# mjmyt/drone_path_planning_python

Hardware: AMD Instinct MI355X
Metric: minimum-snap trajectories/sec (N drones × M segments, order 7) at 1/2/4/8 MI355X (higher is better)
Workload: dtype f64

## Files before the change

### drone_path_planning_python_amd/csrc/msnap_aux.hip

```cpp
#include <math.h>

#include <cstdlib>

#include "msnap_internal.h"

namespace msnap {

__global__ void __launch_bounds__(256)
pack_kernel(const double *__restrict__ coef, const double *__restrict__ dur, float *__restrict__ out,
            size_t n_rows , int nc) {
  const int ncol = 1 + 4 * nc;
  const size_t total = n_rows * (size_t)ncol;
  for (size_t idx = (size_t)blockIdx.x * blockDim.x + threadIdx.x; idx < total;
       idx += (size_t)gridDim.x * blockDim.x) {
    const size_t row = idx / ncol;
    const int col = (int)(idx - row * ncol);
    const double v = (col == 0) ? dur[row] : coef[row * (size_t)(4 * nc) + (col - 1)];
    out[idx] = (float)v;
  }
}

int launch_pack(msnap_ctx *ctx, int n_drones, int n_seg, const double *coef, const double *dur, float *out) {
  const size_t rows = (size_t)n_drones * n_seg;
  const int nc = ctx->order + 1;
// ... 1262 lines not shown
        if (keep && pos < cg.cap) {
          const int a = a0 + ai, b = a + t * kSelThreads + threadIdx.x;
          cg.glist[pos] = (a << 16) | b;
          if (b != a) cg.blist[(size_t)b * cg.nG + a] = pos + 1;
        }
      }
    return;
  }
  constexpr int GPB = kRowBlock / kColBlock;
  constexpr int NW = kSelThreads / kWave;
  __shared__ int wsum[kSelTrips][NW];
  __shared__ int sStart;
  __shared__ double sRow[GPB][8];
  __shared__ double sAll[8];
  const int I = blockIdx.x, lane = threadIdx.x & (kWave - 1), w = threadIdx.x / kWave;
  const int nsh = (N - I * kRowBlock + kColBlock - 1) / kColBlock;
  const int ng = nsh < GPB ? nsh : GPB;
  if (threadIdx.x < 7 * GPB) {
    const int q = threadIdx.x / 7, k = threadIdx.x % 7;
    if (q < ng) sRow[q][k] = k < 6 ? (kStage ? sBox[(I * GPB + q) * 6 + k] : cu.colbox[(size_t)(I * GPB + q) * 6 + k]) : sCmax[I * GPB + q];
  }
  __syncthreads();
  if (threadIdx.x < 7) {
    const int k = threadIdx.x;
    double v = sRow[0][k];
    for (int q = 1; q < ng; ++q) v = k < 3 ? fmin(v, sRow[q][k]) : fmax(v, sRow[q][k]);
    sAll[k] = v;
  }
  __syncthreads();
  unsigned long long mk[kSelTrips];
  bool keep[kSelTrips];
  double cbx[kSelTrips][6], cmx[kSelTrips];
#pragma unroll
  for (int t = 0; t < kSelTrips; ++t) {
    if (t * kSelThreads >= nsh) continue;
    const int k = t * kSelThreads + threadIdx.x, J = I * GPB + (k < nsh ? k : nsh - 1);
    load_box(J, cbx[t]);
    cmx[t] = sCmax[J];
  }
#pragma unroll
  for (int t = 0; t < kSelTrips; ++t) {
    const int k = t * kSelThreads + threadIdx.x;
    keep[t] = false;
    if (k < nsh) {
      keep[t] = true;
      if (k >= GPB) {
        const double cm = cmx[t];
        bool any = false;
        const double lb0 = box_box_lb2(sAll, cbx[t]);
        if (!((lb0 > sAll[6]) & (lb0 > cm))) {
          for (int q = 0; q < ng; ++q) {
            const double lb2 = box_box_lb2(sRow[q], cbx[t]);
            any |= !((lb2 > sRow[q][6]) & (lb2 > cm));
          }
        }
        keep[t] = any;
      }
    }
    mk[t] = __ballot(keep[t]);
    if (lane == 0) wsum[t][w] = __popcll(mk[t]);
  }
  __syncthreads();
  int all = 0, off[kSelTrips];
#pragma unroll
  for (int t = 0; t < kSelTrips; ++t) {
#pragma unroll
    for (int q = 0; q < NW; ++q) {
      if (q == w) off[t] = all;
      all += wsum[t][q];
    }
  }
  if (threadIdx.x == 0) {
    const int start = atomicAdd(&meta[kMetaTotal], all);
    sStart = start;
    meta[kMetaStart + I] = start;
    cnt[I] = all;
  }
  __syncthreads();
#pragma unroll
  for (int t = 0; t < kSelTrips; ++t)
    if (keep[t]) list[sStart + off[t] + __popcll(mk[t] & ((1ull << lane) - 1ull))] = (I << 16) | (t * kSelThreads + threadIdx.x);
}

__device__ __forceinline__ void
collide_span_list_body(const double *__restrict__ prow_t, const double *__restrict__ pcol, CollideGeom g,
                       double *__restrict__ part_d2, int32_t *__restrict__ part_j, double *__restrict__ cpart_d2,
                       int32_t *__restrict__ cpart_i, const int32_t *__restrict__ oid, const int32_t *__restrict__ list,
                       int sp_force, int slots, int32_t *__restrict__ meta) {
  constexpr int CB = kColBlock;
  __shared__ double sFold[CB * kWave];
  __shared__ int sFoldI[CB * kWave];
  const int lane = threadIdx.x;
  const int tot = meta[kMetaTotal];
  const CullSplit sp = cull_split(tot, slots, cull_nch(g.S), sp_force);
  if (blockIdx.x == 0 && lane == 0) {
    meta[kMetaParts] = sp.lo;
    meta[kMetaParts + 1] = sp.hi;
    meta[kMetaParts + 2] = sp.x;
  }
  const int items = sp.items(tot);
  const int xi = sp.x * sp.hi;
  auto share_of = [&](int it) { return it < xi ? it / sp.hi : sp.x + (it - xi) / sp.lo; };
  int it = blockIdx.x;
  int entry = it < items ? list[share_of(it)] : 0;
  while (it < items) {
    const int f = share_of(it);
    g.sparts = it < xi ? sp.hi : sp.lo;
    const int h = it - sp.item_of(f);
    const int I = entry >> 16, k = entry & 0xffff;
    const int nxt = it + gridDim.x;
    entry = nxt < items ? list[share_of(nxt)] : 0;
    const int crow = I * sp.hi + h;
    const int cj = I * kRowBlock + k * CB;
    const int ncols = g.Cn - cj < CB ? g.Cn - cj : CB;
    const bool two_sided = k >= kRowBlock / CB;
    RowSet rs;
#pragma unroll
    for (int rr = 0; rr < kRowsPerLane; ++rr) {
      const int raw = I * kRowBlock + rr * kWave + lane;
      rs.live[rr] = raw < g.R;
      rs.grow[rr] = rs.live[rr] ? raw : g.R - 1;
      rs.best[rr] = INFINITY;
      rs.bestj[rr] = -1;
    }
    const double *prowT = prow_t + (size_t)I * kRowBlock;
    if (ncols <= 2)
      collide_block<2, true>(g, prowT, pcol, cj, ncols, two_sided, rs, I, h, crow, lane, sFold, sFoldI, cpart_d2, cpart_i, oid);
    else if (ncols <= CB / 2)
      collide_block<CB / 2, true>(g, prowT, pcol, cj, ncols, two_sided, rs, I, h, crow, lane, sFold, sFoldI, cpart_d2, cpart_i, oid);
    else
      collide_block<CB, true>(g, prowT, pcol, cj, ncols, two_sided, rs, I, h, crow, lane, sFold, sFoldI, cpart_d2, cpart_i, oid);
#pragma unroll
    for (int rr = 0; rr < kRowsPerLane; ++rr) {
      part_d2[(size_t)it * kRowBlock + rr * kWave + lane] = rs.best[rr];
      part_j[(size_t)it * kRowBlock + rr * kWave + lane] = (rs.best[rr] == INFINITY) ? -1 : rs.bestj[rr];
    }
    it = nxt;
  }
}

constexpr int kGroupHalf = kColBlock / 2;
constexpr int kGroupLanes = kWave / 2;

constexpr int kFinishWaves = 4;
template <int kChunks>
__global__ void __launch_bounds__(kWave * kFinishWaves)
collide_finish_groups_kernel(int N, const int32_t *__restrict__ oid, const int32_t *__restrict__ meta, CullGroups cg,
                             double radius, double *__restrict__ min_dist, int32_t *__restrict__ partner,
                             int32_t *__restrict__ hit) {
  __shared__ int sItAll[kFinishWaves][kChunks * kWave];
  const int lane = threadIdx.x & (kWave - 1), w = __builtin_amdgcn_readfirstlane(threadIdx.x / kWave);
  int *sIt = sItAll[w];
  const int gq = blockIdx.x * kFinishWaves + w;
  if (gq >= cg.nG || meta[kMetaGroups] > cg.cap) return;
  int pl[kChunks];
#pragma unroll
  for (int c = 0; c < kChunks; ++c)
    pl[c] = (c * kWave < gq && c * kWave + lane < gq) ? cg.blist[(size_t)gq * cg.nG + c * kWave + lane] : 0;
  const int nA = cg.acnt[gq], sA = cg.astart[gq];
  const int k = lane & (kColBlock - 1), e = lane >> 3;
  const int r = gq * kColBlock + k;
  const int out = r < N ? oid[r] : 0;
  int nB = 0;
#pragma unroll
  for (int c = 0; c < kChunks; ++c) {
    const unsigned long long m = __ballot(pl[c] > 0);
    if (pl[c] > 0) sIt[nB + __popcll(m & ((1ull << lane) - 1ull))] = pl[c] - 1;
    nB += __popcll(m);
  }
  __builtin_amdgcn_fence(__ATOMIC_RELEASE, "wavefront", "local");
  __builtin_amdgcn_wave_barrier();
  __builtin_amdgcn_fence(__ATOMIC_ACQUIRE, "wavefront", "local");
  double best = INFINITY;
  int bj = -1;
  constexpr int U = 8;
  for (int q0 = 0; q0 < nA + nB; q0 += U * (kWave / kColBlock)) {
    double d[U];
    int j[U];
#pragma unroll
    for (int u = 0; u < U; ++u) {
      const int q = q0 + u * (kWave / kColBlock) + e;
      d[u] = INFINITY;
      j[u] = -1;
      if (q < nA + nB) {
        const size_t slot = (q < nA ? (size_t)(sA + q) * 16 : (size_t)sIt[q - nA] * 16 + kColBlock) + k;
        d[u] = cg.cand_d2[slot];
        j[u] = cg.cand_j[slot];
      }
    }
#pragma unroll
    for (int u = 0; u < U; ++u)
      if (j[u] >= 0 && (bj < 0 || d[u] < best || (d[u] == best && j[u] < bj))) {
        best = d[u];
        bj = j[u];
      }
  }
#pragma unroll
  for (int m = kColBlock; m < kWave; m <<= 1) {
    const double o = shfl_xor_f64(best, m);
    const int oj = __shfl_xor(bj, m);
    if (oj >= 0 && (bj < 0 || o < best || (o == best && oj < bj))) {
      best = o;
      bj = oj;
    }
  }
  if (e == 0 && r < N) {
    const double dist = sqrt(bj >= 0 ? best : INFINITY);
    min_dist[out] = dist;
    partner[out] = bj;
    hit[out] = (dist < 2.0 * radius) ? 1 : 0;
  }
#pragma unroll
  for (int c = 0; c < kChunks; ++c)
    if (pl[c] > 0) cg.blist[(size_t)gq * cg.nG + c * kWave + lane] = 0;
}

constexpr int kGroupWaves = 4;
__global__ void __launch_bounds__(kWave, kGroupWaves)
collide_eval_groups_kernel(const double *__restrict__ pcol, int N, int S, const int32_t *__restrict__ oid,
                           const int32_t *__restrict__ meta, CullGroups cg, unsigned long long *__restrict__ hint) {
#pragma clang fp contract(off)
  const int lane = threadIdx.x;
  int tot = meta[kMetaGroups];
  if (blockIdx.x == 0 && lane == 0 && hint != nullptr)
    __hip_atomic_store(hint, cull_hint_pack(N, meta[kMetaTotal], tot), __ATOMIC_RELAXED, __HIP_MEMORY_SCOPE_SYSTEM);
  if (tot > cg.cap) tot = 0;
  const unsigned stride = (unsigned)S * 3u;
  const int per = (tot + 7) >> 3;
  auto item_of = [&](int v) { return (v >> 3) < per ? (v & 7) * per + (v >> 3) : tot; };
  int v = blockIdx.x, it = item_of(v);
  int entry = (it < tot && it < cg.cap) ? cg.glist[it] : 0;
  for (; (v >> 3) < per; v += gridDim.x, it = item_of(v)) {
    const int it_next = item_of(v + (int)gridDim.x);
    const int ent_raw = entry;
    entry = it_next < tot ? cg.glist[it_next] : 0;
    if (it >= tot) continue;
    const int ent = __builtin_amdgcn_readfirstlane(ent_raw);
    const int a = ent >> 16, b = ent & 0xffff;
    const bool diag = a == b;

    int lane_s = threadIdx.x;
    asm volatile("" : "+v"(lane_s));
    const int half = lane_s >> 5, ls = lane_s & (kGroupLanes - 1);
    double acc[kColBlock * kGroupHalf];
#pragma unroll
    for (int p = 0; p < kColBlock * kGroupHalf; ++p) acc[p] = INFINITY;
#pragma unroll 1
    for (int s0 = 0; s0 < S; s0 += kGroupLanes) {
      const int sq = s0 + ls < S ? s0 + ls : S - 1;
      const unsigned voff = (unsigned)sq * 24u;
      double cx[kGroupHalf], cy[kGroupHalf], cz[kGroupHalf];
#pragma unroll
      for (int c = 0; c < kGroupHalf; ++c) {
        const int d = b * kColBlock + half * kGroupHalf + c;
        const double *p = reinterpret_cast<const double *>(
            reinterpret_cast<const char *>(pcol + (size_t)(d < N ? d : N - 1) * stride) + (size_t)voff);
        cx[c] = p[0];
        cy[c] = p[1];
        cz[c] = p[2];
      }
      double rw[3][3];
      auto fetch = [&](int r, double(&dst)[3]) {
        const int d = a * kColBlock + r;
        const double *p = reinterpret_cast<const double *>(
            reinterpret_cast<const char *>(pcol + (size_t)(d < N ? d : N - 1) * stride) + (size_t)voff);
        dst[0] = p[0];
        dst[1] = p[1];
        dst[2] = p[2];
      };
      fetch(0, rw[0]);
      fetch(1, rw[1]);
#pragma unroll
      for (int r = 0; r < kColBlock; ++r) {
        if (r + 2 < kColBlock) fetch(r + 2, rw[(r + 2) % 3]);
        asm volatile("" ::: "memory");
        const double x = rw[r % 3][0], y = rw[r % 3][1], z = rw[r % 3][2];
#pragma unroll
        for (int c = 0; c < kGroupHalf; ++c) {
          const double dx = cx[c] - x, dy = cy[c] - y, dz = cz[c] - z;
          const double d2 = __builtin_fma(dz, dz, __builtin_fma(dy, dy, dx * dx));
          asm("v_min_f64 %0, %1, %0" : "+v"(acc[r * kGroupHalf + c]) : "v"(d2));
        }
      }
    }
#pragma unroll
    for (int n = 16, m = 16; n >= 1; n >>= 1, m >>= 1) {
      const bool up = (lane_s & m) != 0;
#pragma unroll
      for (int i = 0; i < n; ++i) {
        const double keep = up ? acc[i + n] : acc[i], send = up ? acc[i] : acc[i + n];
        acc[i] = __builtin_fmin(keep, __shfl_xor(send, m));
      }
    }
    double v = acc[0];
    int lane_c = threadIdx.x;
    asm volatile("" : "+v"(lane_c));
    const int pr = (lane_c & (kGroupLanes - 1)) >> 2, pc = lane_c & (kGroupHalf - 1), half_c = lane_c >> 5;
    const int ra = a * kColBlock + pr, cb = b * kColBlock + half_c * kGroupHalf + pc;
    const int oi = oid[ra < N ? ra : N - 1], oj = oid[cb < N ? cb : N - 1];
    if (ra >= N || cb >= N || (diag && ra == cb)) v = INFINITY;
    {
      double w = v;
      int wj = oj;
#pragma unroll
      for (int m = 1; m <= 32; m = (m == 2 ? 32 : m << 1)) {
        const double o = __shfl_xor(w, m);
        const int ojx = __shfl_xor(wj, m);
        const bool take = (o < w) | ((o == w) & (ojx < wj));
        w = take ? o : w;
        wj = take ? ojx : wj;
      }
      if ((lane & 35) == 0) {
        cg.cand_d2[(size_t)it * 16 + pr] = w;
        cg.cand_j[(size_t)it * 16 + pr] = w < INFINITY ? wj : -1;
      }
    }
    {
      double w = v;
      int wi = oi;
#pragma unroll
      for (int m = 4; m <= 16; m <<= 1) {
        const double o = __shfl_xor(w, m);
        const int oix = __shfl_xor(wi, m);
        const bool take = (o < w) | ((o == w) & (oix < wi));
        w = take ? o : w;
        wi = take ? oix : wi;
      }
      if ((lane_c & (kGroupLanes - 1)) < kGroupHalf) {
        const int k = kColBlock + half_c * kGroupHalf + pc;
        cg.cand_d2[(size_t)it * 16 + k] = w;
        cg.cand_j[(size_t)it * 16 + k] = (!diag && w < INFINITY) ? wi : -1;
      }
    }
  }
}

__global__ void __launch_bounds__(kWave, 4)
collide_eval_shares_kernel(const double *__restrict__ prow_t, const double *__restrict__ pcol, CollideGeom g,
                           double *__restrict__ part_d2, int32_t *__restrict__ part_j, double *__restrict__ cpart_d2,
                           int32_t *__restrict__ cpart_i, const int32_t *__restrict__ oid, const int32_t *__restrict__ list,
                           int sp_force, int slots, int32_t *__restrict__ meta, unsigned long long *__restrict__ hint,
                           int groups_cap) {
  if (groups_cap > 0 && meta[kMetaGroups] <= groups_cap) return;
  if (blockIdx.x == 0 && threadIdx.x == 0 && hint != nullptr)
    __hip_atomic_store(hint, cull_hint_pack(g.R, meta[kMetaTotal], meta[kMetaGroups]), __ATOMIC_RELAXED,
                       __HIP_MEMORY_SCOPE_SYSTEM);
  collide_span_list_body(prow_t, pcol, g, part_d2, part_j, cpart_d2, cpart_i, oid, list, sp_force, slots, meta);
}

__global__ void __launch_bounds__(kWave)
collide_short_kernel(const double *__restrict__ prow, const double *__restrict__ pcol, int R, int ro, int Cn, int S,
                     double radius, double *__restrict__ min_dist, int32_t *__restrict__ partner,
                     int32_t *__restrict__ hit, int raw) {
#pragma clang fp contract(off)
  const int r = blockIdx.x * kWave + threadIdx.x;
  if (r >= R) return;
  const int grow = ro + r;
  const double *pr = prow + (size_t)r * S * 3;
  double best = INFINITY;
  int bestj = -1;
  for (int j = 0; j < Cn; ++j) {
    const double *pc = pcol + (size_t)j * S * 3;
    double m = INFINITY;
    for (int sq = 0; sq < S; ++sq) {
      const double dx = pc[(size_t)sq * 3 + 0] - pr[(size_t)sq * 3 + 0];
      const double dy = pc[(size_t)sq * 3 + 1] - pr[(size_t)sq * 3 + 1];
      const double dz = pc[(size_t)sq * 3 + 2] - pr[(size_t)sq * 3 + 2];
      const double d2 = __builtin_fma(dz, dz, __builtin_fma(dy, dy, dx * dx));
      m = __builtin_fmin(d2, m);
    }
    if (j == grow) m = INFINITY;
    if (m < best) {
      best = m;
      bestj = j;
    }
  }
  if (raw) {
    min_dist[r] = best;
    partner[r] = (best == INFINITY) ? -1 : bestj;
    return;
  }
  const double dist = sqrt(best);
  min_dist[r] = dist;
  partner[r] = (best == INFINITY) ? -1 : bestj;
  hit[r] = (dist < 2.0 * radius) ? 1 : 0;
}

constexpr int kMergeRows = 16;
constexpr int kMergeParts = 16;
__global__ void __launch_bounds__(kMergeRows * kMergeParts)
collide_merge_kernel(const double *__restrict__ part_d2, const int32_t *__restrict__ part_j, CollideGeom g,
                     const double *__restrict__ cpart_d2, const int32_t *__restrict__ cpart_i, double radius,
                     double *__restrict__ min_dist, int32_t *__restrict__ partner, int32_t *__restrict__ hit,
                     const int32_t *__restrict__ oid, const int32_t *__restrict__ cnt, const int32_t *__restrict__ meta,
                     int groups_cap = 0) {
  if (groups_cap > 0 && meta[kMetaGroups] <= groups_cap) return;
  __shared__ double sD[kMergeParts][kMergeRows];
  __shared__ int sJ[kMergeParts][kMergeRows];
  const int lr = threadIdx.x & (kMergeRows - 1), q = threadIdx.x / kMergeRows;
  const int r_raw = blockIdx.x * kMergeRows + lr;
  const int r = r_raw < g.R ? r_raw : g.R - 1;
  const int out = oid ? oid[r] : r;
  double best = INFINITY;
  int bj = -1;
  constexpr int U = 8;
  auto sweep = [&](const double *pd, const int32_t *pj, size_t pitch, int n) {
    for (int s0 = q; s0 < n; s0 += U * kMergeParts) {
      double v[U];
      int j[U];
#pragma unroll
      for (int k = 0; k < U; ++k) {
        const int sidx = s0 + k * kMergeParts;
        const int sc = sidx < n ? sidx : n - 1;
        v[k] = pd[(size_t)sc * pitch];
        j[k] = sidx < n ? pj[(size_t)sc * pitch] : -1;
      }
#pragma unroll
      for (int k = 0; k < U; ++k) {
        if (j[k] >= 0 && (v[k] < best || (v[k] == best && j[k] < bj))) {
          best = v[k];
          bj = j[k];
        }
      }
    }
  };
  if (cnt) {
    const int I = __builtin_amdgcn_readfirstlane(r / kRowBlock);
    CullSplit sp;
    sp.lo = meta[kMetaParts];
    sp.hi = meta[kMetaParts + 1];
    sp.x = meta[kMetaParts + 2];
    const int f0 = meta[kMetaStart + I], first_item = sp.item_of(f0), n_items = sp.item_of(f0 + cnt[I]) - first_item;
    const size_t first = (size_t)first_item * kRowBlock + (r - I * kRowBlock);
    sweep(part_d2 + first, part_j + first, kRowBlock, n_items);
    if (I > 0) sweep(cpart_d2 + r, cpart_i + r, (size_t)g.R, I * sp.hi);
  } else if (g.total > 0) {
    const int I = r / kRowBlock;
    long long ua = collide_ustart(g, I), ub = collide_ustart(g, I + 1) - 1;
    ua = ua < g.u_lo ? g.u_lo : ua;
    ub = ub >= g.u_lo + g.u_n ? g.u_lo + g.u_n - 1 : ub;
    if (ub >= ua) {
      const long long wf = collide_share_of(g, ua), wl = collide_share_of(g, ub);
      const size_t first = ((size_t)wf + (I - g.I_lo)) * g.sparts * kRowBlock + (r - I * kRowBlock);
      sweep(part_d2 + first, part_j + first, kRowBlock, (int)(wl - wf + 1) * g.sparts);
    }
    const int Ib = I < g.I_hi + 1 ? I : g.I_hi + 1;
    if (g.sym && Ib > g.I_lo) sweep(cpart_d2 + r, cpart_i + r, (size_t)g.R, (Ib - g.I_lo) * g.sparts);
  }
  sD[q][lr] = best;
  sJ[q][lr] = bj;
  __syncthreads();
  if (q == 0 && r_raw < g.R) {
#pragma unroll
    for (int k = 1; k < kMergeParts; ++k) {
      const double v = sD[k][lr];
      const int j = sJ[k][lr];
      if (j >= 0 && (v < best || (v == best && j < bj))) {
        best = v;
        bj = j;
      }
    }
    if (g.part) {
      min_dist[r] = best;
      partner[r] = bj;
    } else {
      const double dist = sqrt(best);
      min_dist[out] = dist;
      partner[out] = bj;
      hit[out] = (dist < 2.0 * radius) ? 1 : 0;
    }
  }
}

__global__ void __launch_bounds__(256)
collide_finish_kernel(const unsigned char *__restrict__ parts, size_t part_stride, int n_parts, int N, int row_offset,
                      int n_rows, double radius, double *__restrict__ min_dist, int32_t *__restrict__ partner,
                      int32_t *__restrict__ hit) {
  const int i = blockIdx.x * 256 + threadIdx.x;
  if (i >= n_rows) return;
  const int r = row_offset + i;
  double best = INFINITY;
  int bj = -1;
  for (int p = 0; p < n_parts; ++p) {
    const unsigned char *base = parts + (size_t)p * part_stride;
    const double v = reinterpret_cast<const double *>(base)[r];
    const int j = reinterpret_cast<const int32_t *>(base + (size_t)N * sizeof(double))[r];
    if (j >= 0 && (v < best || (v == best && j < bj))) {
      best = v;
      bj = j;
    }
  }
  const double dist = sqrt(best);
  min_dist[i] = dist;
  partner[i] = bj;
  hit[i] = (dist < 2.0 * radius) ? 1 : 0;
}

__global__ void __launch_bounds__(256) collide_part_clear_kernel(double *__restrict__ d2, int32_t *__restrict__ pj, int N) {
  const int i = blockIdx.x * 256 + threadIdx.x;
  if (i < N) {
    d2[i] = INFINITY;
    pj[i] = -1;
  }
}

template <int CTRL>
__device__ __forceinline__ double dpp_f64(double v) {
  const int lo = __builtin_amdgcn_mov_dpp(__double2loint(v), CTRL, 0xF, 0xF, true);
  const int hi = __builtin_amdgcn_mov_dpp(__double2hiint(v), CTRL, 0xF, 0xF, true);
  return __hiloint2double(hi, lo);
}
template <bool MAX>
__device__ __forceinline__ double wave_minmax_f64(double v) {
  auto fold = [](double a, double b) { return MAX ? ((b > a) ? b : a) : ((b < a) ? b : a); };
  v = fold(v, dpp_f64<0xB1>(v));
  v = fold(v, dpp_f64<0x4E>(v));
  v = fold(v, dpp_f64<0x141>(v));
  v = fold(v, dpp_f64<0x140>(v));
  v = fold(v, __shfl_xor(v, 16));
  v = fold(v, __shfl_xor(v, 32));
  return v;
}
__device__ __forceinline__ double wave_min_f64(double v) { return wave_minmax_f64<false>(v); }
__device__ __forceinline__ double wave_max_f64(double v) { return wave_minmax_f64<true>(v); }
template <bool MAX>
__device__ __forceinline__ double wave_minmax_num_f64(double v) {
  auto fold = [](double a, double b) { return MAX ? __builtin_fmax(a, b) : __builtin_fmin(a, b); };
  v = fold(v, dpp_f64<0xB1>(v));
  v = fold(v, dpp_f64<0x4E>(v));
  v = fold(v, dpp_f64<0x141>(v));
  v = fold(v, dpp_f64<0x140>(v));
  v = fold(v, __shfl_xor(v, 16));
  v = fold(v, __shfl_xor(v, 32));
  return v;
}

__device__ __forceinline__ double uniform_f64(double v) {
  return __hiloint2double(__builtin_amdgcn_readfirstlane(__double2hiint(v)),
                          __builtin_amdgcn_readfirstlane(__double2loint(v)));
}


__global__ void __launch_bounds__(kWave * kKeyDrones)
collide_key_kernel(const double *__restrict__ pos, int N, int S, double *__restrict__ box, unsigned *__restrict__ key) {
  const int lane = threadIdx.x & (kWave - 1);
  const int d = blockIdx.x * kKeyDrones + __builtin_amdgcn_readfirstlane(threadIdx.x / kWave);
  if (d >= N) return;
  const double *p = pos + (size_t)d * S * 3;
  double lo[3] = {INFINITY, INFINITY, INFINITY}, hi[3] = {-INFINITY, -INFINITY, -INFINITY};
  const int E = S * 3;
  for (int e0 = 0; e0 < E; e0 += 3 * kWave) {
#pragma unroll
    for (int q = 0; q < 3; ++q) {
      const int e = e0 + q * kWave + lane;
      const double v = e < E ? p[e] : __builtin_nan("");
      const int k = (lane + q) % 3;
      if (__builtin_isfinite(v)) {
#pragma unroll
        for (int kk = 0; kk < 3; ++kk)
          if (k == kk) {
            lo[kk] = v < lo[kk] ? v : lo[kk];
            hi[kk] = v > hi[kk] ? v : hi[kk];
          }
      }
    }
  }
#pragma unroll
  for (int k = 0; k < 3; ++k) {
    lo[k] = uniform_f64(wave_minmax_f64<false>(lo[k]));
    hi[k] = uniform_f64(wave_minmax_f64<true>(hi[k]));
  }
  if (lane < 3) {
    box[(size_t)d * 6 + lane] = lane == 0 ? lo[0] : lane == 1 ? lo[1] : lo[2];
    box[(size_t)d * 6 + 3 + lane] = lane == 0 ? hi[0] : lane == 1 ? hi[1] : hi[2];
  }
  if (lane == 0) key[d] = drone_sort_key(lo, hi);
}

constexpr int kRankWaves = 16;
constexpr int kRankTile = 16;
template <int kRankKeys>
__global__ void __launch_bounds__(kWave * kRankWaves)
collide_rank_kernel(const unsigned *__restrict__ key, int N, int32_t *__restrict__ perm, const double *__restrict__ box,
                    unsigned long long *__restrict__ bound, int32_t *__restrict__ zero, int n_zero,
                    int32_t *__restrict__ meta) {
  __shared__ int cnt[kRankWaves][kRankTile];
  {
    const int gid = blockIdx.x * (kWave * kRankWaves) + threadIdx.x;
    for (int z = gid; z < n_zero; z += gridDim.x * (kWave * kRankWaves)) zero[z] = 0;
    if (gid == 0) {
      meta[kMetaTotal] = 0;
      meta[kMetaGroups] = 0;
    }
  }
  const int lane = threadIdx.x & (kWave - 1), w = __builtin_amdgcn_readfirstlane(threadIdx.x / kWave);
  const int nq = (N + kRankWaves * kWave - 1) / (kRankWaves * kWave);
  const int i0 = blockIdx.x * kRankTile;
  unsigned kraw[kRankKeys];
#pragma unroll
  for (int q = 0; q < kRankKeys; ++q) {
    const int j = (w * nq + q) * kWave + lane;
    kraw[q] = key[(q < nq && j < N) ? j : 0];
  }
  const unsigned ktile = key[i0 + (lane & (kRankTile - 1)) < N ? i0 + (lane & (kRankTile - 1)) : N - 1];
  double bx[6] = {0.0, 0.0, 0.0, 0.0, 0.0, 0.0};
  if (threadIdx.x < kRankTile && i0 + (int)threadIdx.x < N) {
#pragma unroll
    for (int k = 0; k < 6; ++k) bx[k] = box[(size_t)(i0 + threadIdx.x) * 6 + k];
  }
  unsigned long long mine[kRankKeys];
#pragma unroll
  for (int q = 0; q < kRankKeys; ++q) {
    const int j = (w * nq + q) * kWave + lane;
    mine[q] = (q < nq && j < N) ? ((unsigned long long)kraw[q] << 32) | (unsigned)j : ~0ull;
  }
#pragma unroll
  for (int t = 0; t < kRankTile; ++t) {
    const int i = i0 + t < N ? i0 + t : N - 1;
    const unsigned long long ki = ((unsigned long long)(unsigned)__builtin_amdgcn_readlane((int)ktile, t) << 32) | (unsigned)i;
    int c = 0;
#pragma unroll
    for (int q = 0; q < kRankKeys; ++q)
      if (q < nq) c += __popcll(__ballot(mine[q] < ki));
    if (lane == 0) cnt[w][t] = c;
  }
  lds_barrier();
  if (threadIdx.x < kRankTile && i0 + (int)threadIdx.x < N) {
    int r = 0;
#pragma unroll
    for (int q = 0; q < kRankWaves; ++q) r += cnt[q][threadIdx.x];
    const int i = i0 + threadIdx.x;
    perm[r] = i;
    const bool has = (bx[0] <= bx[3]) & (bx[1] <= bx[4]) & (bx[2] <= bx[5]);
    bound[r] = has ? 0x7ff0000000000000ull : 0ull;
  }
}

#ifndef MSNAP_TILE_E
#define MSNAP_TILE_E 15
#endif
constexpr int kTileE = MSNAP_TILE_E, kTileRows = 64, kTileHalo = 4;
constexpr int kTilePitch = kTileE + 1 + (kTileE & 1);
static_assert(kTileE % 3 == 0, "whole samples per tile");
constexpr int kBoxGroups = 32;
__global__ void __launch_bounds__(256)
collide_gather_kernel(const double *__restrict__ pos, int N, int Rp, int E, double *__restrict__ prow_t,
                      double *__restrict__ psorted, const int32_t *__restrict__ perm, unsigned long long *__restrict__ bound,
                      const double *__restrict__ box, double *__restrict__ colbox, int nx, int ny, int n_box,
                      int32_t *__restrict__ fill, size_t fill_n) {
#pragma clang fp contract(off)
  __shared__ double tile[(kTileRows + kTileHalo) * kTilePitch];
  __shared__ double sF[kTileHalo][kTileRows];
  const int tid = threadIdx.x;
  const int nb = (int)blockIdx.x - nx * ny;
  if (nb >= n_box) {
    const size_t stride = (size_t)(gridDim.x - nx * ny - n_box) * 256;
    for (size_t i = (size_t)(nb - n_box) * 256 + tid; i < fill_n; i += stride) fill[i] = -1;
    return;
  }
  if (nb >= 0) {
    const int gq = nb * kBoxGroups + (tid >> 3), r = gq * kColBlock + (tid & 7);
    double g6[6];
#pragma unroll
    for (int k = 0; k < 6; ++k) g6[k] = k < 3 ? INFINITY : -INFINITY;
    if (r < N) {
      const double *bx = box + (size_t)perm[r] * 6;
#pragma unroll
      for (int k = 0; k < 6; ++k) g6[k] = bx[k];
    }
#pragma unroll
    for (int k = 0; k < 6; ++k) {
      auto fold = [k](double a, double c) { return k < 3 ? fmin(a, c) : fmax(a, c); };
      g6[k] = fold(g6[k], dpp_f64<0xB1>(g6[k]));
      g6[k] = fold(g6[k], dpp_f64<0x4E>(g6[k]));
      g6[k] = fold(g6[k], dpp_f64<0x141>(g6[k]));
    }
    if ((tid & 7) == 0 && gq * kColBlock < N) {
#pragma unroll
      for (int k = 0; k < 6; ++k) colbox[(size_t)gq * 6 + k] = g6[k];
    }
    return;
  }
  const int bx = blockIdx.x % nx, by = blockIdx.x / nx;
  const int r0 = bx * kTileRows, e0 = by * kTileE;
  const int ne = E - e0 < kTileE ? E - e0 : kTileE;
  __shared__ int sPerm[kTileRows + kTileHalo];
  if (tid < kTileRows + kTileHalo) sPerm[tid] = perm[r0 + tid < N ? r0 + tid : N - 1];
  __syncthreads();
  constexpr int kElems = (kTileRows + kTileHalo) * kTileE, kPer = (kElems + 255) / 256;
  double val[kPer];
#pragma unroll
  for (int u = 0; u < kPer; ++u) {
    const int idx = tid + u * 256, i = idx / kTileE, tx = idx - i * kTileE;
    val[u] = (idx < kElems && tx < ne) ? pos[(size_t)sPerm[i] * E + e0 + tx] : 0.0;
  }
#pragma unroll
  for (int u = 0; u < kPer; ++u) {
    const int idx = tid + u * 256, i = idx / kTileE, tx = idx - i * kTileE;
    if (idx < kElems) {
      tile[i * kTilePitch + tx] = val[u];
      if (i < kTileRows && tx < ne && r0 + i < N) psorted[(size_t)(r0 + i) * E + e0 + tx] = val[u];
    }
  }
  lds_barrier();
  {
    const int tx = tid & 63, ty = tid >> 6;
    for (int i = ty; i < ne; i += 4) prow_t[(size_t)(e0 + i) * Rp + r0 + tx] = tile[tx * kTilePitch + i];
  }
  {
    const int row = tid & 63, k = (tid >> 6) + 1;
    const double *pa = tile + row * kTilePitch, *pb = tile + (row + k) * kTilePitch;
    double f = INFINITY;
    for (int q = 0; q < ne; q += 3) {
      const double dx = pb[q] - pa[q], dy = pb[q + 1] - pa[q + 1], dz = pb[q + 2] - pa[q + 2];
      f = __builtin_fmin(__builtin_fma(dz, dz, __builtin_fma(dy, dy, dx * dx)), f);
    }
    sF[k - 1][row] = r0 + row + k < N ? f : INFINITY;
  }
  lds_barrier();
  if (tid < kTileRows + kTileHalo) {
    double b = INFINITY;
#pragma unroll
    for (int k = 1; k <= kTileHalo; ++k) {
      if (tid < kTileRows) b = __builtin_fmin(b, sF[k - 1][tid]);
      if (tid >= k && tid - k < kTileRows) b = __builtin_fmin(b, sF[k - 1][tid - k]);
    }
    if (b < INFINITY && r0 + tid < N) atomicMin(&bound[r0 + tid], (unsigned long long)__double_as_longlong(b));
  }
}

bool collide_counts_by_groups(const msnap_ctx *ctx, int n_drones, int shares_surviving, int group_pairs_surviving) {
  if (ctx->collide_cull_mode == 1) return false;
  if (n_drones > kCullGroupMaxDrones && 2LL * group_pairs_surviving > kGroupCapLarge) return false;
  if (ctx->collide_cull_mode == 2) return true;
  return cull_groups_cheaper(shares_surviving, group_pairs_surviving);
}

bool formation_collide_takes_broad_phase(const msnap_ctx *ctx, int n_rows, int row_offset, int n_cols, int n_samples) {
  if (n_samples < kSampleChunk || n_rows != n_cols || row_offset != 0 || ctx->collide_no_cull || ctx->collide_no_sym) return false;
  const int cull_min = ctx->collide_cull_min_drones > 0 ? ctx->collide_cull_min_drones : kCullMinDrones;
  return n_rows >= cull_min && n_rows >= 2 * kRowBlock && n_rows <= kCullMaxDrones;
}

int launch_formation_collide(msnap_ctx *ctx, int n_rows, int row_offset, int n_cols, int n_samples,
                             const double *pos_rows, const double *pos_cols, double radius, double *min_dist,
                             int32_t *partner, int32_t *hit, const double *rows_t_in) {
  CollideGeom g;
  g.R = n_rows;
  g.ro = row_offset;
  g.Cn = n_cols;
  g.S = n_samples;
  g.n_rb = (n_rows + kRowBlock - 1) / kRowBlock;
  g.Rp = g.n_rb * kRowBlock;
  g.sparts = 1;
  g.u_lo = 0;
  g.u_n = 0;
  g.I_lo = 0;
  g.I_hi = g.n_rb - 1;
  g.part = 0;
  if (n_cols == 0) {
    g.os = g.oe = 0;
    g.sym = 0;
    g.upw = g.upw_tail = 1;
    g.split = 0;
    g.total = 0;
    hipLaunchKernelGGL(collide_merge_kernel, dim3((n_rows + kMergeRows - 1) / kMergeRows), dim3(kMergeRows * kMergeParts), 0, ctx->stream,
                       (const double *)nullptr, (const int32_t *)nullptr, g, (const double *)nullptr,
                       (const int32_t *)nullptr, radius, min_dist, partner, hit, (const int32_t *)nullptr,
                       (const int32_t *)nullptr, (const int32_t *)nullptr);
    MSNAP_HIP(ctx, hipGetLastError());
    return MSNAP_OK;
  }
  if (n_samples < kSampleChunk) {
    hipLaunchKernelGGL(collide_short_kernel, dim3((n_rows + kWave - 1) / kWave), dim3(kWave), 0, ctx->stream,
                       pos_rows, pos_cols, n_rows, row_offset, n_cols, n_samples, radius, min_dist, partner, hit, 0);
    MSNAP_HIP(ctx, hipGetLastError());
    return MSNAP_OK;
  }
  const bool rows_in_cols = (long long)row_offset + n_rows <= n_cols;
  g.os = rows_in_cols ? row_offset : n_cols;
  g.oe = rows_in_cols ? row_offset + n_rows : n_cols;
  const size_t cpart_entries = (size_t)g.n_rb * n_rows;
  g.sym = (rows_in_cols && n_rows > kRowBlock && !ctx->collide_no_sym && cpart_entries * 12 <= ((size_t)2 << 30)) ? 1 : 0;
  ctx->collide_last_sym = g.sym;
  g.upw = 1;
  g.total = collide_ustart(g, g.n_rb);
  g.u_n = g.total;
  long long upw = kColBlock;
  const long long slots = (long long)ctx->n_cu * 4 * 4;
  if (ctx->collide_waves_per_cu > 0) {
    upw = g.total / ((long long)ctx->n_cu * ctx->collide_waves_per_cu) / kColBlock * kColBlock;
    if (upw < kColBlock) upw = kColBlock;
  }
  long long waves;
  while (((g.total + upw - 1) / upw + g.n_rb) * kRowBlock * 12 > ((long long)512 << 20)) upw *= 2;
  g.upw = (int)upw;
  g.upw_tail = (int)upw;
  g.split = (g.total + upw - 1) / upw * upw;
  const long long shares = (g.total + upw - 1) / upw;
  if (upw == kColBlock && ctx->collide_waves_per_cu == 0 && shares <= slots && n_rows == n_cols) {
    g.upw_tail = kColBlock / 2;
    g.split = shares * 3 / 4 * upw;
  } else if (upw == kColBlock && ctx->collide_waves_per_cu == 0 && shares % slots != 0 && shares % slots <= slots / 8) {
    g.upw_tail = 2;
    g.split = (shares - shares % slots) * upw;
  }
  waves = g.split / upw + (g.total - g.split + g.upw_tail - 1) / g.upw_tail;
  const bool cull = g.sym && formation_collide_takes_broad_phase(ctx, n_rows, row_offset, n_cols, n_samples);
  ctx->collide_last_cull = 0;
  ctx->collide_meta = nullptr;
  ctx->collide_last_shares = (int)(waves < 0x7fffffff ? waves : 0x7fffffff);
  const int E = n_samples * 3;
  if (cull) {
    const int N = n_rows;
    const size_t nJ = ((size_t)N + kColBlock - 1) / kColBlock;
    long long shares = 0;
    for (int I = 0; I < g.n_rb; ++I) shares += (N - I * kRowBlock + kColBlock - 1) / kColBlock;
    const long long all_groups = (long long)nJ * (nJ + 1) / 2;
    const bool all_fit = N <= kCullGroupMaxDrones;
    bool by_groups = false;
    if (ctx->collide_cull_mode == 2) {
      by_groups = true;
    } else if (ctx->collide_cull_mode != 1 && ctx->cull_hint) {
      const unsigned long long h = *(volatile unsigned long long *)ctx->cull_hint;
      const int hN = (int)(h >> 48) & 0x7fff;
      const long long hs = (long long)((h >> 24) & 0xffffff), hg = (long long)(h & 0xffffff);
      by_groups = h != 0 && hN == (N & 0x7fff) && hg != 0xffffff && cull_groups_cheaper(hs, hg) &&
                  (all_fit || 2 * hg <= kGroupCapLarge);
    }
    const bool both = by_groups && !all_fit;
    const int spmax = N > 8192 ? 2 : kCullMaxParts;
    ctx->collide_last_shares = (int)shares;
    const int sp_force = (ctx->collide_sample_parts > 0 ? (ctx->collide_sample_parts < spmax ? ctx->collide_sample_parts : spmax) : 0) |
                         (spmax << 8);
    const long long items_max = (sp_force & 0xff) ? shares * (sp_force & 0xff) : (shares > 2 * slots ? shares : 2 * slots);
    const size_t entries = (by_groups && !both) ? 0 : (size_t)items_max * kRowBlock;
    const size_t centries = (by_groups && !both) ? 0 : (size_t)g.n_rb * spmax * N;
    const size_t gcap = !by_groups ? 0 : all_fit ? (size_t)all_groups : (size_t)kGroupCapLarge;
    const bool have_keys = handover_form(ctx, rows_t_in, N, n_samples) == 2;
    const size_t doubles = (size_t)g.Rp * E + (size_t)N * E + (size_t)N * 6 + nJ * 6 + (size_t)N + entries + centries + gcap * 16;
    const size_t ints = entries + centries + (size_t)N + (size_t)N + (size_t)shares + g.n_rb + kMetaWords + 2 * nJ + gcap +
                        gcap * 16 + (by_groups ? nJ * nJ : 0);
    int rc = ensure(ctx, ctx->stage[7], doubles * sizeof(double) + ints * sizeof(int32_t) + 64);
    if (rc) return rc;
    double *rows_t = (double *)ctx->stage[7].p;
    double *psorted = rows_t + (size_t)g.Rp * E, *box_own = psorted + (size_t)N * E, *colbox = box_own + (size_t)N * 6;
    unsigned long long *bound = (unsigned long long *)(colbox + nJ * 6);
    double *pd = (double *)(bound + N), *cd = pd + entries;
    double *cand_d2 = cd + centries;
    int32_t *pj = (int32_t *)(cand_d2 + gcap * 16), *ci = pj + entries;
    unsigned *key_own = (unsigned *)(ci + centries);
    int32_t *perm = (int32_t *)(key_own + N), *surv = perm + N, *cnt = surv + shares, *meta = cnt + g.n_rb;
    int32_t *acnt = meta + kMetaWords, *astart = acnt + nJ;
    int32_t *blist = astart + nJ, *glist = blist + (by_groups ? nJ * nJ : 0), *cand_j = glist + gcap;
    const double *box = have_keys ? rows_t_in : box_own;
    const unsigned *key = have_keys ? reinterpret_cast<const unsigned *>(rows_t_in + (size_t)N * 6) : key_own;
    CullGroups cg{glist, astart, acnt, blist, cand_d2, cand_j, (int)gcap, (int)nJ};
    const bool trust = by_groups && !stream_is_capturing(ctx) && !ctx->stage[7].in_graph;
    const bool blist_clean = trust && ctx->blist_clean == (const void *)blist && ctx->blist_clean_n == (int)nJ;
    ctx->blist_clean = trust ? (const void *)blist : nullptr;
    ctx->blist_clean_n = (int)nJ;
    ctx->collide_meta = meta;
    ctx->collide_last_cull = 1;
    ctx->collide_last_by_groups = by_groups ? (all_fit ? 1 : 2) : 0;
    ctx->collide_last_n = N;
    if (!have_keys) {
      hipLaunchKernelGGL(collide_key_kernel, dim3((N + kKeyDrones - 1) / kKeyDrones), dim3(kWave * kKeyDrones), 0,
                         ctx->stream, pos_cols, N, n_samples, box_own, key_own);
      MSNAP_HIP(ctx, hipGetLastError());
    }
    hipLaunchKernelGGL((N <= 4096 ? collide_rank_kernel<4> : N <= 8192 ? collide_rank_kernel<8> : collide_rank_kernel<16>),
                       dim3((N + kRankTile - 1) / kRankTile), dim3(kWave * kRankWaves), 0, ctx->stream, key, N, perm, box,
                       bound, blist, (int)(by_groups && !blist_clean ? nJ * nJ : 0), meta);
    MSNAP_HIP(ctx, hipGetLastError());
    const int nx = g.Rp / kTileRows, ny = (E + kTileE - 1) / kTileE;
    const int n_box = (int)((nJ + kBoxGroups - 1) / kBoxGroups), n_fill = centries ? 4 * nx : 0;
    hipLaunchKernelGGL(collide_gather_kernel, dim3((unsigned)(nx * ny + n_box + n_fill)), dim3(256), 0, ctx->stream, pos_cols, N,
                       g.Rp, E, rows_t, psorted, (const int32_t *)perm, bound, box, colbox, nx, ny, n_box, ci, centries);
    MSNAP_HIP(ctx, hipGetLastError());
    CollideCull cu{colbox};
    hipLaunchKernelGGL((N <= kCullGroupMaxDrones ? collide_select_kernel<1> : collide_select_kernel<2>),
                       dim3(g.n_rb + (unsigned)((nJ + kSelGroups - 1) / kSelGroups)), dim3(kSelThreads), 0, ctx->stream, N, g.n_rb, cu,
                       (const double *)bound, surv, cnt, meta, cg);
    MSNAP_HIP(ctx, hipGetLastError());
    if (by_groups) {
      hipLaunchKernelGGL(collide_eval_groups_kernel, dim3((unsigned)(ctx->n_cu * 4 * kGroupWaves)), dim3(kWave), 0, ctx->stream,
                         (const double *)psorted, N, n_samples, (const int32_t *)perm, (const int32_t *)meta, cg, ctx->cull_hint);
      MSNAP_HIP(ctx, hipGetLastError());
      hipLaunchKernelGGL((N <= 4096 ? collide_finish_groups_kernel<8> : N <= 8192 ? collide_finish_groups_kernel<16> : collide_finish_groups_kernel<32>),
                         dim3((unsigned)((nJ + kFinishWaves - 1) / kFinishWaves)),
                         dim3(kWave * kFinishWaves), 0, ctx->stream, N, (const int32_t *)perm, (const int32_t *)meta, cg, radius,
                         min_dist, partner, hit);
      MSNAP_HIP(ctx, hipGetLastError());
      if (!both) return MSNAP_OK;
    }
    hipLaunchKernelGGL(collide_eval_shares_kernel, dim3((unsigned)slots), dim3(kWave), 0, ctx->stream, (const double *)rows_t,
                       (const double *)psorted, g, pd, pj, cd, ci, (const int32_t *)perm, (const int32_t *)surv, sp_force,
                       (int)slots, meta, ctx->cull_hint, both ? (int)gcap : 0);
    MSNAP_HIP(ctx, hipGetLastError());
    hipLaunchKernelGGL(collide_merge_kernel, dim3((N + kMergeRows - 1) / kMergeRows), dim3(kMergeRows * kMergeParts), 0,
                       ctx->stream, pd, pj, g, cd, ci, radius, min_dist, partner, hit, (const int32_t *)perm,
                       (const int32_t *)cnt, (const int32_t *)meta, both ? (int)gcap : 0);
    MSNAP_HIP(ctx, hipGetLastError());
    return MSNAP_OK;
  }
  if (handover_form(ctx, rows_t_in, n_rows, n_samples) != 1) rows_t_in = nullptr;
  if (ctx->collide_sample_parts > 0) {
    g.sparts = ctx->collide_sample_parts < 8 ? ctx->collide_sample_parts : 8;
  } else if (ctx->collide_waves_per_cu == 0) {
    const int nch = (n_samples + kSampleChunk - 1) / kSampleChunk;
    while (g.sparts < 8 && waves * g.sparts < slots / 4 && nch / (g.sparts * 2) >= 2) g.sparts *= 2;
  }
  if (upw > 0x3fffffff || waves * g.sparts > 0x7fffffff) return MSNAP_EINVAL;
  const size_t part_entries = ((size_t)waves + g.n_rb) * g.sparts * kRowBlock;
  const size_t centries = g.sym ? cpart_entries * g.sparts : 0;
  const size_t t_entries = rows_t_in ? 0 : (size_t)g.Rp * E;
  ctx->blist_clean = nullptr;
  int rc = ensure(ctx, ctx->stage[7],
                  t_entries * sizeof(double) + (part_entries + centries) * (sizeof(double) + sizeof(int32_t)) + 64);
  if (rc) return rc;
  double *rows_t = (double *)ctx->stage[7].p;
  double *pd = rows_t + t_entries;
  double *cd = pd + part_entries;
  int32_t *pj = (int32_t *)(cd + centries);
  int32_t *ci = pj + part_entries;
  if (!rows_t_in) {
    hipLaunchKernelGGL(collide_transpose_kernel, dim3(g.Rp / 64, (E + 31) / 32), dim3(256), 0, ctx->stream, pos_rows,
                       n_rows, g.Rp, E, rows_t, (E + 31) / 32, (int32_t *)nullptr, (size_t)0, (const int32_t *)nullptr,
                       (double *)nullptr);
    MSNAP_HIP(ctx, hipGetLastError());
  }
  hipLaunchKernelGGL(collide_span_kernel, dim3((unsigned)(waves * g.sparts)), dim3(kWave), 0, ctx->stream,
                     rows_t_in ? rows_t_in : (const double *)rows_t, pos_cols, g, pd, pj, cd, ci);
  MSNAP_HIP(ctx, hipGetLastError());
  hipLaunchKernelGGL(collide_merge_kernel, dim3((n_rows + kMergeRows - 1) / kMergeRows), dim3(kMergeRows * kMergeParts), 0,
                     ctx->stream, pd, pj, g, cd, ci, radius, min_dist, partner, hit, (const int32_t *)nullptr,
                     (const int32_t *)nullptr, (const int32_t *)nullptr);
  MSNAP_HIP(ctx, hipGetLastError());
  return MSNAP_OK;
}

int launch_formation_collide_part(msnap_ctx *ctx, int N, int n_samples, const double *pos_all, int part, int n_parts,
                                  double *out_d2, int32_t *out_j) {
  if (n_samples < kSampleChunk) {
    const int r0 = (int)((long long)N * part / n_parts), r1 = (int)((long long)N * (part + 1) / n_parts);
    hipLaunchKernelGGL(collide_part_clear_kernel, dim3((N + 255) / 256), dim3(256), 0, ctx->stream, out_d2, out_j, N);
    MSNAP_HIP(ctx, hipGetLastError());
    if (r1 > r0) {
      hipLaunchKernelGGL(collide_short_kernel, dim3((r1 - r0 + kWave - 1) / kWave), dim3(kWave), 0, ctx->stream,
                         pos_all + (size_t)r0 * n_samples * 3, pos_all, r1 - r0, r0, N, n_samples, 0.0, out_d2 + r0,
                         out_j + r0, (int32_t *)nullptr, 1);
      MSNAP_HIP(ctx, hipGetLastError());
    }
    return MSNAP_OK;
  }
  CollideGeom g;
  g.R = N;
  g.ro = 0;
  g.Cn = N;
  g.S = n_samples;
  g.n_rb = (N + kRowBlock - 1) / kRowBlock;
  g.os = 0;
  g.oe = N;
  g.sym = 1;
  g.total = collide_ustart(g, g.n_rb);
  auto cut = [&](int p) {
    const long long u = g.total * p / n_parts / kColBlock * kColBlock;
    return p >= n_parts ? g.total : u;
  };
  g.u_lo = cut(part);
  g.u_n = cut(part + 1) - g.u_lo;
  g.part = 1;
  g.sparts = 1;
  g.upw = g.upw_tail = kColBlock;
  g.I_lo = 0;
  g.I_hi = -1;
  const long long shares = (g.u_n + kColBlock - 1) / kColBlock;
  g.split = shares * kColBlock;
  long long waves = shares;
  if (shares > 0) {
    const long long u0 = g.u_lo, u1 = g.u_lo + g.u_n - 1;
    while (g.I_lo + 1 < g.n_rb && collide_ustart(g, g.I_lo + 1) <= u0) ++g.I_lo;
    g.I_hi = g.I_lo;
    while (g.I_hi + 1 < g.n_rb && collide_ustart(g, g.I_hi + 1) <= u1) ++g.I_hi;
    const long long slots = (long long)ctx->n_cu * 4 * 4;
    const int nch = (n_samples + kSampleChunk - 1) / kSampleChunk;
    if (ctx->collide_sample_parts > 0) {
      g.sparts = ctx->collide_sample_parts < 8 ? ctx->collide_sample_parts : 8;
    } else if (shares * 2 <= slots) {
      long long sp = slots / shares;
      sp = sp > 8 ? 8 : sp;
      while (sp > 1 && nch / sp < 2) --sp;
      g.sparts = (int)sp;
    } else if (shares % slots != 0 && shares % slots <= slots / 8 && shares > slots) {
      g.upw_tail = 2;
      g.split = (shares - shares % slots) * kColBlock;
    }
    waves = g.split / kColBlock + (g.u_n - g.split + g.upw_tail - 1) / g.upw_tail;
  }
  const int nrb = g.I_hi - g.I_lo + 1;
  g.Rp = (nrb > 0 ? nrb : 1) * kRowBlock;
  if (waves * g.sparts > 0x7fffffff) return MSNAP_EINVAL;
  const size_t part_entries = ((size_t)waves + (size_t)(nrb > 0 ? nrb : 0)) * g.sparts * kRowBlock;
  const size_t centries = (size_t)(nrb > 0 ? nrb : 0) * g.sparts * (size_t)N;
  const int E = n_samples * 3;
  const size_t t_entries = (size_t)g.Rp * E;
  if ((part_entries + centries) * 12 > ((size_t)16 << 30)) return MSNAP_ENOMEM;
  ctx->collide_last_cull = 0;
  ctx->collide_meta = nullptr;
  ctx->blist_clean = nullptr;
  int rc = ensure(ctx, ctx->stage[7],
                  t_entries * sizeof(double) + (part_entries + centries) * (sizeof(double) + sizeof(int32_t)) + 64);
  if (rc) return rc;
  double *rows_t = (double *)ctx->stage[7].p;
  double *pd = rows_t + t_entries;
  double *cd = pd + part_entries;
  int32_t *pj = (int32_t *)(cd + centries);
  int32_t *ci = pj + part_entries;
  if (waves > 0) {
    const int r_first = g.I_lo * kRowBlock;
    const int r_cnt = (N - r_first) < g.Rp ? (N - r_first) : g.Rp;
    const int ny = (E + 31) / 32;
    hipLaunchKernelGGL(collide_transpose_kernel, dim3(g.Rp / 64, ny + 4), dim3(256), 0, ctx->stream,
                       pos_all + (size_t)r_first * E, r_cnt, g.Rp, E, rows_t, ny, ci, centries, (const int32_t *)nullptr,
                       (double *)nullptr);
    MSNAP_HIP(ctx, hipGetLastError());
    hipLaunchKernelGGL(collide_span_kernel, dim3((unsigned)(waves * g.sparts)), dim3(kWave), 0, ctx->stream,
                       (const double *)rows_t, pos_all, g, pd, pj, cd, ci);
    MSNAP_HIP(ctx, hipGetLastError());
  } else {
    g.total = 0;
  }
  hipLaunchKernelGGL(collide_merge_kernel, dim3((N + kMergeRows - 1) / kMergeRows), dim3(kMergeRows * kMergeParts), 0,
                     ctx->stream, pd, pj, g, cd, ci, 0.0, out_d2, out_j, (int32_t *)nullptr, (const int32_t *)nullptr,
                     (const int32_t *)nullptr, (const int32_t *)nullptr);
  MSNAP_HIP(ctx, hipGetLastError());
  return MSNAP_OK;
}

int launch_formation_collide_finish(msnap_ctx *ctx, int N, int n_parts, const void *parts, size_t part_stride,
// ... 292 lines not shown
```

Before: 58.86 million.

## Read unsorted positions via permutation in group eval, skip sorted copies

In the group-based collision path, the eval kernel now reads positions directly from the original column buffer through the rank permutation instead of from a pre-sorted copy. The permutation entries for the next work item are prefetched. The gather kernel is templated so the sorted-row and transposed copies are skipped when only the group path runs, and the workspace shrinks to match. The permutation array is padded to whole groups so the eval kernel needs no bounds clamps. The finish kernel now also clears its blist row when the group capacity overflows. This removes a full write and re-read of the position data, at the cost of indirect, less coalesced loads in eval.

```diff
diff --git a/drone_path_planning_python_amd/csrc/msnap_aux.hip b/drone_path_planning_python_amd/csrc/msnap_aux.hip
--- a/drone_path_planning_python_amd/csrc/msnap_aux.hip
+++ b/drone_path_planning_python_amd/csrc/msnap_aux.hip
@@ -1438,11 +1438,20 @@
   const int lane = threadIdx.x & (kWave - 1), w = __builtin_amdgcn_readfirstlane(threadIdx.x / kWave);
   int *sIt = sItAll[w];
   const int gq = blockIdx.x * kFinishWaves + w;
-  if (gq >= cg.nG || meta[kMetaGroups] > cg.cap) return;
+  if (gq >= cg.nG) return;
   int pl[kChunks];
 #pragma unroll
   for (int c = 0; c < kChunks; ++c)
     pl[c] = (c * kWave < gq && c * kWave + lane < gq) ? cg.blist[(size_t)gq * cg.nG + c * kWave + lane] : 0;
+  auto clear_row = [&] {
+#pragma unroll
+    for (int c = 0; c < kChunks; ++c)
+      if (pl[c] > 0) cg.blist[(size_t)gq * cg.nG + c * kWave + lane] = 0;
+  };
+  if (meta[kMetaGroups] > cg.cap) {
+    clear_row();
+    return;
+  }
   const int nA = cg.acnt[gq], sA = cg.astart[gq];
   const int k = lane & (kColBlock - 1), e = lane >> 3;
   const int r = gq * kColBlock + k;
@@ -1496,14 +1505,12 @@
     partner[out] = bj;
     hit[out] = (dist < 2.0 * radius) ? 1 : 0;
   }
-#pragma unroll
-  for (int c = 0; c < kChunks; ++c)
-    if (pl[c] > 0) cg.blist[(size_t)gq * cg.nG + c * kWave + lane] = 0;
+  clear_row();
 }
 
 constexpr int kGroupWaves = 4;
 __global__ void __launch_bounds__(kWave, kGroupWaves)
-collide_eval_groups_kernel(const double *__restrict__ pcol, int N, int S, const int32_t *__restrict__ oid,
+collide_eval_groups_kernel(const double *__restrict__ pos, int N, int S, const int32_t *__restrict__ oid,
                            const int32_t *__restrict__ meta, CullGroups cg, unsigned long long *__restrict__ hint) {
 #pragma clang fp contract(off)
   const int lane = threadIdx.x;
@@ -1516,6 +1523,17 @@
   auto item_of = [&](int v) { return (v >> 3) < per ? (v & 7) * per + (v >> 3) : tot; };
   int v = blockIdx.x, it = item_of(v);
   int entry = (it < tot && it < cg.cap) ? cg.glist[it] : 0;
+  auto perm_of = [&](int ent_raw, int(&dst)[2 * kColBlock]) {
+    const int ent = __builtin_amdgcn_readfirstlane(ent_raw);
+    const int32_t *pa = oid + (ent >> 16) * kColBlock, *pb = oid + (ent & 0xffff) * kColBlock;
+#pragma unroll
+    for (int r = 0; r < kColBlock; ++r) {
+      dst[r] = pa[r];
+      dst[kColBlock + r] = pb[r];
+    }
+  };
+  int prm[2 * kColBlock];
+  perm_of(entry, prm);
   for (; (v >> 3) < per; v += gridDim.x, it = item_of(v)) {
     const int it_next = item_of(v + (int)gridDim.x);
     const int ent_raw = entry;
@@ -1538,18 +1556,17 @@
       double cx[kGroupHalf], cy[kGroupHalf], cz[kGroupHalf];
 #pragma unroll
       for (int c = 0; c < kGroupHalf; ++c) {
-        const int d = b * kColBlock + half * kGroupHalf + c;
+        const int d = half ? prm[kColBlock + kGroupHalf + c] : prm[kColBlock + c];
         const double *p = reinterpret_cast<const double *>(
-            reinterpret_cast<const char *>(pcol + (size_t)(d < N ? d : N - 1) * stride) + (size_t)voff);
+            reinterpret_cast<const char *>(pos + (size_t)d * stride) + (size_t)voff);
         cx[c] = p[0];
         cy[c] = p[1];
         cz[c] = p[2];
       }
       double rw[3][3];
       auto fetch = [&](int r, double(&dst)[3]) {
-        const int d = a * kColBlock + r;
         const double *p = reinterpret_cast<const double *>(
-            reinterpret_cast<const char *>(pcol + (size_t)(d < N ? d : N - 1) * stride) + (size_t)voff);
+            reinterpret_cast<const char *>(pos + (size_t)prm[r] * stride) + (size_t)voff);
         dst[0] = p[0];
         dst[1] = p[1];
         dst[2] = p[2];
@@ -1569,6 +1586,9 @@
         }
       }
     }
+    int prm_next[2 * kColBlock];
+    perm_of(entry, prm_next);
+    asm volatile("" ::: "memory");
 #pragma unroll
     for (int n = 16, m = 16; n >= 1; n >>= 1, m >>= 1) {
       const bool up = (lane_s & m) != 0;
@@ -1618,6 +1638,8 @@
         cg.cand_j[(size_t)it * 16 + k] = (!diag && w < INFINITY) ? wi : -1;
       }
     }
+#pragma unroll
+    for (int r = 0; r < 2 * kColBlock; ++r) prm[r] = prm_next[r];
   }
 }
 
@@ -1874,6 +1896,7 @@
   {
     const int gid = blockIdx.x * (kWave * kRankWaves) + threadIdx.x;
     for (int z = gid; z < n_zero; z += gridDim.x * (kWave * kRankWaves)) zero[z] = 0;
+    if (gid < ((-N) & (kColBlock - 1))) perm[N + gid] = 0;
     if (gid == 0) {
       meta[kMetaTotal] = 0;
       meta[kMetaGroups] = 0;
@@ -1929,6 +1952,7 @@
 constexpr int kTilePitch = kTileE + 1 + (kTileE & 1);
 static_assert(kTileE % 3 == 0, "whole samples per tile");
 constexpr int kBoxGroups = 32;
+template <bool kCopies>
 __global__ void __launch_bounds__(256)
 collide_gather_kernel(const double *__restrict__ pos, int N, int Rp, int E, double *__restrict__ prow_t,
                       double *__restrict__ psorted, const int32_t *__restrict__ perm, unsigned long long *__restrict__ bound,
@@ -1985,11 +2009,11 @@
     const int idx = tid + u * 256, i = idx / kTileE, tx = idx - i * kTileE;
     if (idx < kElems) {
       tile[i * kTilePitch + tx] = val[u];
-      if (i < kTileRows && tx < ne && r0 + i < N) psorted[(size_t)(r0 + i) * E + e0 + tx] = val[u];
+      if (kCopies && i < kTileRows && tx < ne && r0 + i < N) psorted[(size_t)(r0 + i) * E + e0 + tx] = val[u];
     }
   }
   lds_barrier();
-  {
+  if constexpr (kCopies) {
     const int tx = tid & 63, ty = tid >> 6;
     for (int i = ty; i < ne; i += 4) prow_t[(size_t)(e0 + i) * Rp + r0 + tx] = tile[tx * kTilePitch + i];
   }
@@ -2124,19 +2148,22 @@
     const size_t centries = (by_groups && !both) ? 0 : (size_t)g.n_rb * spmax * N;
     const size_t gcap = !by_groups ? 0 : all_fit ? (size_t)all_groups : (size_t)kGroupCapLarge;
     const bool have_keys = handover_form(ctx, rows_t_in, N, n_samples) == 2;
-    const size_t doubles = (size_t)g.Rp * E + (size_t)N * E + (size_t)N * 6 + nJ * 6 + (size_t)N + entries + centries + gcap * 16;
-    const size_t ints = entries + centries + (size_t)N + (size_t)N + (size_t)shares + g.n_rb + kMetaWords + 2 * nJ + gcap +
+    const bool copies = !by_groups || both;
+    const size_t img = copies ? (size_t)g.Rp * E : 0, cols = copies ? (size_t)N * E : 0;
+    const size_t doubles = img + cols + (size_t)N * 6 + nJ * 6 + (size_t)N + entries + centries + gcap * 16;
+    const size_t ints = entries + centries + (size_t)N + nJ * kColBlock + (size_t)shares + g.n_rb + kMetaWords + 2 * nJ + gcap +
                         gcap * 16 + (by_groups ? nJ * nJ : 0);
     int rc = ensure(ctx, ctx->stage[7], doubles * sizeof(double) + ints * sizeof(int32_t) + 64);
     if (rc) return rc;
-    double *rows_t = (double *)ctx->stage[7].p;
-    double *psorted = rows_t + (size_t)g.Rp * E, *box_own = psorted + (size_t)N * E, *colbox = box_own + (size_t)N * 6;
+    double *rows_t = copies ? (double *)ctx->stage[7].p : nullptr;
+    double *psorted = copies ? rows_t + img : nullptr;
+    double *box_own = (double *)ctx->stage[7].p + img + cols, *colbox = box_own + (size_t)N * 6;
     unsigned long long *bound = (unsigned long long *)(colbox + nJ * 6);
     double *pd = (double *)(bound + N), *cd = pd + entries;
     double *cand_d2 = cd + centries;
     int32_t *pj = (int32_t *)(cand_d2 + gcap * 16), *ci = pj + entries;
     unsigned *key_own = (unsigned *)(ci + centries);
-    int32_t *perm = (int32_t *)(key_own + N), *surv = perm + N, *cnt = surv + shares, *meta = cnt + g.n_rb;
+    int32_t *perm = (int32_t *)(key_own + N), *surv = perm + nJ * kColBlock, *cnt = surv + shares, *meta = cnt + g.n_rb;
     int32_t *acnt = meta + kMetaWords, *astart = acnt + nJ;
     int32_t *blist = astart + nJ, *glist = blist + (by_groups ? nJ * nJ : 0), *cand_j = glist + gcap;
     const double *box = have_keys ? rows_t_in : box_own;
@@ -2161,8 +2188,9 @@
     MSNAP_HIP(ctx, hipGetLastError());
     const int nx = g.Rp / kTileRows, ny = (E + kTileE - 1) / kTileE;
     const int n_box = (int)((nJ + kBoxGroups - 1) / kBoxGroups), n_fill = centries ? 4 * nx : 0;
-    hipLaunchKernelGGL(collide_gather_kernel, dim3((unsigned)(nx * ny + n_box + n_fill)), dim3(256), 0, ctx->stream, pos_cols, N,
-                       g.Rp, E, rows_t, psorted, (const int32_t *)perm, bound, box, colbox, nx, ny, n_box, ci, centries);
+    hipLaunchKernelGGL((copies ? collide_gather_kernel<true> : collide_gather_kernel<false>), dim3((unsigned)(nx * ny + n_box + n_fill)),
+                       dim3(256), 0, ctx->stream, pos_cols, N, g.Rp, E, rows_t, psorted, (const int32_t *)perm, bound, box,
+                       colbox, nx, ny, n_box, ci, centries);
     MSNAP_HIP(ctx, hipGetLastError());
     CollideCull cu{colbox};
     hipLaunchKernelGGL((N <= kCullGroupMaxDrones ? collide_select_kernel<1> : collide_select_kernel<2>),
@@ -2171,7 +2199,7 @@
     MSNAP_HIP(ctx, hipGetLastError());
     if (by_groups) {
       hipLaunchKernelGGL(collide_eval_groups_kernel, dim3((unsigned)(ctx->n_cu * 4 * kGroupWaves)), dim3(kWave), 0, ctx->stream,
-                         (const double *)psorted, N, n_samples, (const int32_t *)perm, (const int32_t *)meta, cg, ctx->cull_hint);
+                         pos_cols, N, n_samples, (const int32_t *)perm, (const int32_t *)meta, cg, ctx->cull_hint);
       MSNAP_HIP(ctx, hipGetLastError());
       hipLaunchKernelGGL((N <= 4096 ? collide_finish_groups_kernel<8> : N <= 8192 ? collide_finish_groups_kernel<16> : collide_finish_groups_kernel<32>),
                          dim3((unsigned)((nJ + kFinishWaves - 1) / kFinishWaves)),
```

Result: no change. 58.87 million, median of 6 (+0.0%).
